# facebookresearch/omni3d

Hardware: AMD Instinct MI355X
Metric: images/sec train DLA34_FPN b=4/GPU (higher is better)
Workload: dtype f32; 1 GPU; cubercnn_DLA34_FPN train step, batch 4/GPU, synthetic Omni3D 512x512 (8 GT/img), fwd+10 losses+bwd+allreduce+divergence guard+SGD, random-init weights; global_batch=4, image=512x512, parallelism=dp1 (flat-bucket RCCL all-reduce)

## Files before the change

### include/omni3d_hip.h

```cpp
#ifndef OMNI3D_HIP_H
#define OMNI3D_HIP_H

#ifdef __cplusplus
extern "C" {
#endif


int omni_iou_box3d(const float* boxes1, int N, const float* boxes2, int M, const int* valid1, float* vol,
                   float* iou, int* overflow, void* stream);

int omni_iou_box3d_pairs(const float* boxes1, const float* boxes2, const int* idx1, const int* idx2,
                         long long npairs, const int* valid1, float* vol, float* iou, int* overflow,
                         void* stream);

int omni_iou_box3d_pairs_algo(const float* boxes1, const float* boxes2, const int* idx1, const int* idx2,
                              long long npairs, const int* valid1, float* vol, float* iou, int* overflow,
                              int lanes_per_pair, void* stream);

int omni_box3d_validity(const float* boxes, int N, float eps_coplanar, float eps_nonzero, int* valid,
                        int* counts, void* stream);

int omni_nms3d(const float* verts, const float* score, const int* cls, const int* count, int B, int S, float iou_thr,
               int class_agnostic, float eps_coplanar, float eps_nonzero, float* iou, int* keep, int* order, int* new_count,
               int* overflow, void* stream);
// ... 142 lines not shown


int omni_pairwise_iou(const float* boxes1, int N, const float* boxes2, int M, int mode, float* out, void* stream);


int omni_rpn_finalize_labels(const float* anchors, int A, int B, const int* gt_off, const float* ign,
                             const int* ign_off, const signed char* match_label, const int* gt_best_idx,
                             const float* pos_val, const int* pos_idx, const float* neg_val, const int* neg_idx,
                             int kpos, int kneg, int batch_per_image, float ignore_thresh, signed char* labels,
                             int* counts, void* stream);

int omni_rpn_gather_logits(const void* const* level_ptrs, const int* level_hw, int nlev, int B, float* logits,
                           void* stream);

int omni_rpn_head16_fwd(const void* const* t, const long long* pix, int nlev, const float* w_obj, const float* b_obj,
                        const float* w_del, const float* b_del, const void* const* y, void* stream);
int omni_rpn_head16_dgrad(const void* const* dy, const void* const* t, const long long* pix, int nlev, const float* w_obj,
                          const float* w_del, int relu_mask, const void* const* dt, void* stream);
int omni_rpn_head16_wgrad(const void* const* dy, const void* const* t, const long long* pix, int nlev, float* partial,
                          int partial_rows, float* dw_obj, float* db_obj, float* dw_del, float* db_del, int accumulate, void* stream);

int omni_rpn_loss_fwd(const void* const* level_ptrs, const int* level_hw, int nlev, int B, const float* anchors,
                      const signed char* labels, const int* matched_idx, const float* gt, const int* gt_off,
                      double* sums, void* stream);
int omni_rpn_loss_bwd(const void* const* level_ptrs, const void* const* dlevel_ptrs, const int* level_hw, int nlev,
                      int B, const float* anchors, const signed char* labels, const int* matched_idx,
                      const float* gt, const int* gt_off, const float* g_cls, const float* g_loc, float inv_norm,
                      void* stream);

int omni_rpn_loss_plain_fwd(const void* const* level_ptrs, const int* level_hw, int nlev, int B, const float* anchors,
                            const signed char* labels, const int* matched_idx, const float* gt, const int* gt_off,
                            double* sums, void* stream);
int omni_rpn_loss_plain_bwd(const void* const* level_ptrs, const void* const* dlevel_ptrs, const int* level_hw, int nlev,
                            int B, const float* anchors, const signed char* labels, const int* matched_idx,
                            const float* gt, const int* gt_off, const float* g_cls, const float* g_loc, float inv_norm,
                            void* stream);

int omni_rpn_reg_loss_fwd(const void* const* level_ptrs, const int* level_hw, int nlev, int B, const float* anchors,
                          const signed char* labels, const int* matched_idx, const float* gt, const int* gt_off, int plain,
                          int reg_type, float beta, float scale_clamp, double* sums, void* stream);
int omni_rpn_reg_loss_bwd(const void* const* level_ptrs, const void* const* dlevel_ptrs, const int* level_hw, int nlev,
                          int B, const float* anchors, const signed char* labels, const int* matched_idx,
                          const float* gt, const int* gt_off, int plain, int reg_type, float beta, float scale_clamp,
                          const float* g_cls, const float* g_loc, float inv_norm, void* stream);

int omni_rpn_decode(const void* const* level_ptrs, const int* level_hw, int nlev, int B, int Ktot,
                    const int* slot_level, const int* idx, const float* anchors, const int* image_hw,
                    float scale_clamp, float min_size, float* boxes, int* valid, void* stream);

int omni_rpn_mask_scores(const float* scores, const int* keep, long long n, float* masked, void* stream);
int omni_rpn_collect(const float* boxes, const float* top_v, const int* top_i, int B, int N, int P, float* prop,
                     int* count, void* stream);

int omni_rpn_match_draw(const float* anchors, int A, const float* gt, const int* gt_off, int B, int G, float thr_lo,
                        float thr_hi, int l0, int l1, int l2, int allow_low_quality, const float* expo, long long* draw_state,
                        int* ticket, float eps, float* matched_val, int* matched_idx, signed char* match_label, int* gt_best_bits,
                        int* gt_best_idx, float* key_pos, float* key_neg, void* stream);
int omni_roi_sample_draw(const float* prop_boxes, const int* prop_count, int B, int pmax, const float* gt, const int* gt_cls,
                         const int* gt_off, const float* ign, const int* ign_off, const float* expo, long long* draw_state, int* ticket,
                         float iou_thr, float ignore_thresh, float eps, int num_classes, int batch_per_image, int nfg_max,
                         int append_gt, float* out_boxes, int* out_cls, int* out_gt, float* out_iou, int* out_counts, int* out_row,
                         int first, float* first_boxes, int* first_cls, int* first_row, void* stream);


int omni_roi_levels(const float* rois, int R, int min_level, int max_level, float canonical_size,
                    int canonical_level, int* levels, void* stream);

int omni_roi_align_fwd(const void* const* level_ptrs, const int* level_hw, const float* level_scale, int nlev,
                       const float* rois, const int* batch_idx, const int* levels, int R, int P, int C,
                       float* out, void* stream);
int omni_roi_align_fwd_mode(const void* const* level_ptrs, const int* level_hw, const float* level_scale, int nlev,
                            const float* rois, const int* batch_idx, const int* levels, int R, int P, int C, int aligned, float* out,
                            void* stream);
int omni_roi_align_bwd_mode(const void* const* dlevel_ptrs, const int* level_hw, const float* level_scale, int nlev,
                            const float* rois, const int* batch_idx, const int* levels, int R, int P, int C, int aligned,
                            const float* dout, void* stream);
int omni_roi_pool_fwd(const void* const* level_ptrs, const int* level_hw, const float* level_scale, int nlev, const float* rois,
                      const int* batch_idx, const int* levels, int R, int P, int C, float* out, int* argmax, void* stream);
int omni_roi_pool_bwd(const void* const* dlevel_ptrs, const int* level_hw, const float* level_scale, int nlev, const int* batch_idx,
                      const int* levels, int R, int P, int C, const float* dout, const int* argmax, void* stream);
int omni_roi_align_fwd2(const void* const* level_ptrs, const int* level_hw, const float* level_scale, int nlev,
                        const float* rois, const int* batch_idx, const int* levels, int R, int P, int C, float* out,
                        float* out2, int per_image, int first, void* stream);
int omni_roi_align_bwd(const void* const* dlevel_ptrs, const int* level_hw, const float* level_scale, int nlev,
                       const float* rois, const int* batch_idx, const int* levels, int R, int P, int C,
                       const float* dout, void* stream);
int omni_roi_align_bwd2(const void* const* dlevel_ptrs, const int* level_hw, const float* level_scale, int nlev,
                        const float* rois, const int* batch_idx, const int* levels, int R, int P, int C,
                        const float* dout, const float* dout2, int per_image, int first, void* stream);
int omni_roi_align_bwd_det(const void* const* dlevel_ptrs, const int* level_hw, const float* level_scale, int nlev, int B,
                           const float* rois, const int* batch_idx, const int* levels, int R, int P, int C, const float* dout,
                           const float* dout2, int per_image, int first, float* ws, long long ws_floats, int* ctr, int n_ctr,
                           long long* plan, void* stream);


int omni_box_loss_fwd(const float* pred, int ldp, int R, int K, const int* cls, const float* prop, const float* gt,
                      const int* gt_row, float wx, float wy, float ww, float wh, double* sums, void* stream);
int omni_box_loss_bwd(const float* pred, int ldp, int R, int K, const int* cls, const float* prop, const float* gt,
                      const int* gt_row, float wx, float wy, float ww, float wh, const double* sums,
                      const float* g_cls, const float* g_reg, float* dpred, void* stream);

int omni_box_reg_loss_fwd(const float* pred, int ldp, int R, int K, const int* cls, const float* prop, const float* gt,
                          const int* gt_row, float wx, float wy, float ww, float wh, int reg_type, float beta,
                          float scale_clamp, double* sums, void* stream);
int omni_box_reg_loss_bwd(const float* pred, int ldp, int R, int K, const int* cls, const float* prop, const float* gt,
                          const int* gt_row, float wx, float wy, float ww, float wh, int reg_type, float beta,
                          float scale_clamp, const double* sums, const float* g_cls, const float* g_reg, float* dpred,
                          void* stream);

int omni_box_decode_gt_class(const float* pred, int ldp, int R, int K, const int* cls, const float* prop, float wx, float wy,
                             float ww, float wh, float scale_clamp, float* out, void* stream);

int omni_cube_loss_fwd(const float* head, int ldh, int F, int K, int mode, int bins, const float* zscales, const float* zstats,
                       const float* boxes, const int* cls, const int* img,
                       const float* Ks, const float* v2r, const float* priors, const float* gt3d,
                       const float* gtpose, const int* gt_row, float w_dims, float w_pose, float w_xy, float w_z, float w_joint,
                       float* vals, float* jac, float* red, void* stream);
int omni_cube_loss_bwd(const float* vals, const float* jac, const float* red, const float* gk, const int* cls,
                       const float* boxes, int F, int K, int mode, int bins, const float* zscales, int ldh, float* dhead,
                       void* stream);
int omni_cube_decode(const float* head, int ldh, int F, int K, int mode, int bins, const float* zscales, const float* zstats,
                     const float* boxes, const int* cls, const int* img,
                     const float* Ks, const float* v2r, const float* ratio, const float* priors, float* cube3d,
                     float* pose, float* verts, void* stream);
int omni_cuboid_corners(const float* box3d, const float* R, int n, float* verts, void* stream);

int omni_conv2d_fwd_stats(const float* x, const float* w, float* out, int N, int H, int W, int C, int K, int R, int S,
                          int stride, int pad, int ldx, int ldo, float* stats, int stats_rows, int* nblk_out, void* stream);
int omni_wino_out_stats(const float* M, float* y, int N, int H, int W, int K, int tile, float* stats, int stats_rows,
                        int* nblk_out, void* stream);
int omni_wino_out_bn_bwd_stats(const float* M, float* y, int N, int H, int W, int K, int tile, const float* bn_x,
                               const float* mean_rstd, const float* scale_shift, float* stats, int stats_rows, int* nblk_out,
                               void* stream);
int omni_stem_conv_fwd_stats(const float* x, const float* w, float* out, int N, int H, int W, int C, int K, int R, int ldx,
                             int ldo, float* stats, int stats_rows, int* nblk_out, void* stream);

int omni_gemm_engine(const float* A, const float* B, float* C, const float* bias, int form, int batch, int M, int N, int K,
                     int lda, int ldb, int ldc, long long stride_a, long long stride_b, long long stride_c, int splits,
                     int relu, int accumulate, int tile, int workgroups, void* stream);
int omni_gemm_engine_det(const float* A, const float* B, float* C, const float* bias, int form, int batch, int M, int N, int K,
                         int lda, int ldb, int ldc, long long stride_a, long long stride_b, long long stride_c, int splits,
                         int relu, int accumulate, int tile, int workgroups, float* ws, long long ws_floats, int* ctr, int n_ctr,
                         long long* plan, void* stream);

int omni_transpose2d(const float* src, float* dst, int rows, int cols, void* stream);

int omni_det_scores(const float* pred, int ld, const float* rois, const int* count, const int* image_hw, int B, int P, int K,
                    float wx, float wy, float ww, float wh, float score_thresh, float* scores, float* probs, float* boxes,
                    void* stream);
int omni_det_nms_boxes(const float* boxes, const float* vals, const int* idx, int B, int PK, int K, int cap, float* nms_boxes,
                       int* valid, void* stream);
int omni_det_compact(const int* keep, const int* valid, const float* vals, const int* idx, const float* boxes, int B, int PK,
                     int K, int cap, int topk, float* out_box, float* out_score, int* out_cls, int* out_roi, int* out_count,
                     void* stream);

int omni_resize_bilinear_u8(const unsigned char* src, unsigned char* dst, unsigned char* tmp, int planes, int H, int W,
                            int HO, int WO, const int* bounds_h, const int* kk_h, int ksize_h, const int* bounds_v,
                            const int* kk_v, int ksize_v, int flip, void* stream);


int omni_sgd_step(float* param, const float* grad, float* momentum_buf, long long n, float lr, float momentum,
                  float dampening, float weight_decay, int nesterov, int first_step, float grad_scale,
                  const float* skip_flag, void* stream);
int omni_adam_step(float* param, const float* grad, float* exp_avg, float* exp_avg_sq, float* max_exp_avg_sq, long long n, float lr,
                   float beta1, float beta2, float eps, float weight_decay, int decoupled, const float* step, float grad_scale,
                   const float* skip_flag, void* stream);
// ... 149 lines not shown
```

### omni3d_amd/csrc/roi_align.hip

```cpp
#include <device_rt.h>
#pragma clang fp contract(off)

namespace {

constexpr int MAXL = 8;
struct FeatLevels {
    float* f[MAXL];
    int H[MAXL], W[MAXL];
    float scale[MAXL];
    int nlev;
};

__global__ void roi_levels_kernel(const float* __restrict__ rois, int R, int min_level, int max_level,
                                  float canonical_size, int canonical_level, int* __restrict__ levels) {
    const int r = blockIdx.x * blockDim.x + threadIdx.x;
    if (r >= R) return;
    const float w = rois[4 * r + 2] - rois[4 * r + 0], h = rois[4 * r + 3] - rois[4 * r + 1];
    const float sz = sqrtf(w * h);
    float lv = floorf((float)canonical_level + log2f(sz / canonical_size + 1e-8f));
    lv = fminf(fmaxf(lv, (float)min_level), (float)max_level);
    levels[r] = (int)lv - min_level;
}

struct Tap { int y0, y1, x0, x1; float w00, w01, w10, w11; bool ok; };

__device__ __forceinline__ Tap make_tap(float y, float x, int H, int W) {
    Tap t;
    t.ok = !(y < -1.0f || y > (float)H || x < -1.0f || x > (float)W);
    if (y <= 0.f) y = 0.f;
    if (x <= 0.f) x = 0.f;
    int y_low = (int)y, x_low = (int)x, y_high, x_high;
    if (y_low >= H - 1) { y_high = y_low = H - 1; y = (float)y_low; } else { y_high = y_low + 1; }
    if (x_low >= W - 1) { x_high = x_low = W - 1; x = (float)x_low; } else { x_high = x_low + 1; }
    const float ly = y - (float)y_low, lx = x - (float)x_low, hy = 1.f - ly, hx = 1.f - lx;
    t.y0 = y_low; t.y1 = y_high; t.x0 = x_low; t.x1 = x_high;
    t.w00 = hy * hx; t.w01 = hy * lx; t.w10 = ly * hx; t.w11 = ly * lx;
    return t;
}

template <int DIR>
__global__ void __launch_bounds__(256) roi_align_kernel(FeatLevels fl, const float* __restrict__ rois,
                                                        const int* __restrict__ batch_idx, const int* __restrict__ levels,
                                                        int R, int P, int C, float* __restrict__ out,
                                                        float* __restrict__ out2 = nullptr, int per_image = 0, int first = 0, int aligned = 1) {
    const int wave = threadIdx.x >> 6, lane = threadIdx.x & 63;
    const long job = (long)blockIdx.x * 4 + wave;
    if (job >= (long)R * P * P) return;
    const int r = (int)(job / (P * P)), bin = (int)(job % (P * P));
    const int ph = bin / P, pw = bin % P;
    const int l = levels[r];
    const int H = fl.H[l], W = fl.W[l];
    const float sc = fl.scale[l];
    const float off = aligned ? 0.5f : 0.f;
    const float sw = rois[4 * r + 0] * sc - off, sh = rois[4 * r + 1] * sc - off;
    const float ew = rois[4 * r + 2] * sc - off, eh = rois[4 * r + 3] * sc - off;
    float rw = ew - sw, rh = eh - sh;
    if (!aligned) { rw = fmaxf(rw, 1.f); rh = fmaxf(rh, 1.f); }
    const float bin_h = rh / (float)P, bin_w = rw / (float)P;
    const int gh = (int)ceilf(rh / (float)P), gw = (int)ceilf(rw / (float)P);
    const float count = (float)max(gh * gw, 1);
    float* feat = fl.f[l] + (long)batch_idx[r] * H * W * C;
    float* o = out + job * C;
    if (DIR == 1) {
        for (int c = lane; c < C; c += 64) {
            const float g = o[c] / count;
            for (int iy = 0; iy < gh; ++iy) {
                const float y = sh + (float)ph * bin_h + ((float)iy + 0.5f) * bin_h / (float)gh;
                for (int ix = 0; ix < gw; ++ix) {
                    const float x = sw + (float)pw * bin_w + ((float)ix + 0.5f) * bin_w / (float)gw;
                    const Tap t = make_tap(y, x, H, W);
                    if (!t.ok) continue;
                    atomicAdd(feat + ((long)t.y0 * W + t.x0) * C + c, g * t.w00);
                    atomicAdd(feat + ((long)t.y0 * W + t.x1) * C + c, g * t.w01);
                    atomicAdd(feat + ((long)t.y1 * W + t.x0) * C + c, g * t.w10);
                    atomicAdd(feat + ((long)t.y1 * W + t.x1) * C + c, g * t.w11);
                }
            }
        }
        return;
    }
    const int C4 = C >> 2;
    for (int c4 = lane; c4 < C4; c4 += 64) {
        float4 acc = make_float4(0.f, 0.f, 0.f, 0.f);
        for (int iy = 0; iy < gh; ++iy) {
            const float y = sh + (float)ph * bin_h + ((float)iy + 0.5f) * bin_h / (float)gh;
            for (int ix = 0; ix < gw; ++ix) {
                const float x = sw + (float)pw * bin_w + ((float)ix + 0.5f) * bin_w / (float)gw;
                const Tap t = make_tap(y, x, H, W);
                if (!t.ok) continue;
                const float* p00 = feat + ((long)t.y0 * W + t.x0) * C + 4 * c4;
                const float* p01 = feat + ((long)t.y0 * W + t.x1) * C + 4 * c4;
                const float* p10 = feat + ((long)t.y1 * W + t.x0) * C + 4 * c4;
                const float* p11 = feat + ((long)t.y1 * W + t.x1) * C + 4 * c4;
                const float4 a = *reinterpret_cast<const float4*>(p00), b = *reinterpret_cast<const float4*>(p01);
                const float4 c = *reinterpret_cast<const float4*>(p10), d = *reinterpret_cast<const float4*>(p11);
                acc.x += t.w00 * a.x + t.w01 * b.x + t.w10 * c.x + t.w11 * d.x;
                acc.y += t.w00 * a.y + t.w01 * b.y + t.w10 * c.y + t.w11 * d.y;
                acc.z += t.w00 * a.z + t.w01 * b.z + t.w10 * c.z + t.w11 * d.z;
                acc.w += t.w00 * a.w + t.w01 * b.w + t.w10 * c.w + t.w11 * d.w;
            }
        }
        acc.x /= count; acc.y /= count; acc.z /= count; acc.w /= count;
        *reinterpret_cast<float4*>(o + 4 * c4) = acc;
        if (DIR == 0 && out2 != nullptr && (r % per_image) < first)
            *reinterpret_cast<float4*>(out2 + (((long)(r / per_image) * first + (r % per_image)) * P * P + bin) * C + 4 * c4) = acc;
    }
}

constexpr int SEP_MAXF = 144;

struct Tap1 { int lo, hi; float wlo, whi; bool ok; };
__device__ __forceinline__ Tap1 make_tap1(float v, int L) {
    Tap1 t;
    t.ok = !(v < -1.0f || v > (float)L);
    if (v <= 0.f) v = 0.f;
    int lo = (int)v, hi;
    if (lo >= L - 1) { hi = lo = L - 1; v = (float)lo; } else { hi = lo + 1; }
    const float l = v - (float)lo;
    t.lo = lo; t.hi = hi; t.whi = l; t.wlo = 1.f - l;
    return t;
}

template <int PP>
__global__ void __launch_bounds__(256) roi_align_bwd_sep_kernel(FeatLevels fl, const float* __restrict__ rois,
                                                                const int* __restrict__ batch_idx,
                                                                const int* __restrict__ levels, int R, int C,
                                                                const float* __restrict__ dout, const float* __restrict__ dout2,
                                                                int per_image, int first) {
    __shared__ __attribute__((aligned(16))) float s_w[4][2][SEP_MAXF][8];
    const int wave = threadIdx.x >> 6, lane = threadIdx.x & 63;
    const int CG = (C + 63) / 64;
    const long job = (long)blockIdx.x * 4 + wave;
    const bool live = job < (long)R * CG;
    const int r = live ? (int)(job / CG) : 0, cg = live ? (int)(job % CG) : 0;
    const int c = cg * 64 + lane;
    const int l = levels[r];
    const int H = fl.H[l], W = fl.W[l];
    const float sc = fl.scale[l];
    const float sw = rois[4 * r + 0] * sc - 0.5f, sh = rois[4 * r + 1] * sc - 0.5f;
    const float ew = rois[4 * r + 2] * sc - 0.5f, eh = rois[4 * r + 3] * sc - 0.5f;
    const float rw = ew - sw, rh = eh - sh;
    const float bin_h = rh / (float)PP, bin_w = rw / (float)PP;
    const int gh = (int)ceilf(rh / (float)PP), gw = (int)ceilf(rw / (float)PP);
    const bool any = live && gh > 0 && gw > 0;
    float* feat = fl.f[l] + (long)batch_idx[r] * H * W * C;
    int Y0 = 0, X0 = 0, fh = 0, fw = 0;
    if (any) {
        Y0 = make_tap1(sh + 0.5f * bin_h / (float)gh, H).lo;
        X0 = make_tap1(sw + 0.5f * bin_w / (float)gw, W).lo;
        fh = make_tap1(sh + (float)(PP - 1) * bin_h + ((float)(gh - 1) + 0.5f) * bin_h / (float)gh, H).hi - Y0 + 1;
        fw = make_tap1(sw + (float)(PP - 1) * bin_w + ((float)(gw - 1) + 0.5f) * bin_w / (float)gw, W).hi - X0 + 1;
    }
    const bool sep = any && fh <= SEP_MAXF && fw <= SEP_MAXF;
    float (*wy)[8] = s_w[wave][0];
    float (*wx)[8] = s_w[wave][1];
    if (sep) {
        for (int i = lane; i < fh * 8; i += 64) wy[i >> 3][i & 7] = 0.f;
        for (int i = lane; i < fw * 8; i += 64) wx[i >> 3][i & 7] = 0.f;
    }
    __syncthreads();
    if (sep) {
        if (lane < PP) {
            for (int ix = 0; ix < gw; ++ix) {
                const Tap1 t = make_tap1(sw + (float)lane * bin_w + ((float)ix + 0.5f) * bin_w / (float)gw, W);
                if (!t.ok) continue;
                wx[t.lo - X0][lane] += t.wlo;
                wx[t.hi - X0][lane] += t.whi;
            }
        } else if (lane >= 32 && lane < 32 + PP) {
            const int ph = lane - 32;
            for (int iy = 0; iy < gh; ++iy) {
                const Tap1 t = make_tap1(sh + (float)ph * bin_h + ((float)iy + 0.5f) * bin_h / (float)gh, H);
                if (!t.ok) continue;
                wy[t.lo - Y0][ph] += t.wlo;
                wy[t.hi - Y0][ph] += t.whi;
            }
        }
    }
    __syncthreads();
    if (!any || c >= C) return;
    const float inv_count = 1.f / (float)(gh * gw);
    const float* o = dout != nullptr ? dout + (long)r * PP * PP * C + c : nullptr;
    const float* o2 = nullptr;
    if (dout2 != nullptr) {
        const int img = r / per_image, k = r - img * per_image;
        if (k < first) o2 = dout2 + ((long)img * first + k) * PP * PP * C + c;
    }
    auto gval = [&](int bin) -> float {
        float v = o != nullptr ? o[(long)bin * C] : 0.f;
        if (o2 != nullptr) v += o2[(long)bin * C];
        return v * inv_count;
    };
    if (sep) {
        float g[PP][PP];
#pragma unroll
        for (int ph = 0; ph < PP; ++ph)
#pragma unroll
            for (int pw = 0; pw < PP; ++pw) g[ph][pw] = gval(ph * PP + pw);
        for (int yy = 0; yy < fh; ++yy) {
            float rowT[PP];
#pragma unroll
            for (int pw = 0; pw < PP; ++pw) rowT[pw] = 0.f;
            bool row_any = false;
// ... 212 lines not shown
    if (wave == 0 && cok) {
        float* feat = fl.f[l] + (long)n * H * W * C + c;
#pragma unroll
        for (int yy = 0; yy < GT_TH; ++yy)
#pragma unroll
            for (int xx = 0; xx < GT_TW; ++xx)
                if (ty0 + yy < H && tx0 + xx < W) *reinterpret_cast<float4*>(feat + ((long)(ty0 + yy) * W + tx0 + xx) * C) = acc[yy * GT_TW + xx];
    }
}

FeatLevels make_feat(const void* const* ptrs, const int* hw, const float* scales, int nlev) {
    FeatLevels fl;
    for (int l = 0; l < MAXL; ++l) { fl.f[l] = nullptr; fl.H[l] = fl.W[l] = 0; fl.scale[l] = 0.f; }
    for (int l = 0; l < nlev; ++l) { fl.f[l] = (float*)ptrs[l]; fl.H[l] = hw[2 * l]; fl.W[l] = hw[2 * l + 1]; fl.scale[l] = scales[l]; }
    fl.nlev = nlev;
    return fl;
}

template <int DIR>
__global__ void __launch_bounds__(256) roi_pool_kernel(FeatLevels fl, const float* __restrict__ rois, const int* __restrict__ batch_idx,
                                                       const int* __restrict__ levels, int R, int P, int C, float* __restrict__ out,
                                                       int* __restrict__ argmax) {
    const int wave = threadIdx.x >> 6, lane = threadIdx.x & 63;
    const long job = (long)blockIdx.x * 4 + wave;
    if (job >= (long)R * P * P) return;
    const int r = (int)(job / (P * P)), bin = (int)(job % (P * P));
    const int ph = bin / P, pw = bin % P;
    const int l = levels[r];
    const int H = fl.H[l], W = fl.W[l];
    float* feat = fl.f[l] + (long)batch_idx[r] * H * W * C;
    const int C4 = C >> 2;
    if (DIR == 1) {
        for (int c4 = lane; c4 < C4; c4 += 64) {
            const float4 g = *reinterpret_cast<const float4*>(out + job * C + 4 * c4);
            const int4 a = *reinterpret_cast<const int4*>(argmax + job * C + 4 * c4);
            if (a.x >= 0) atomicAdd(feat + (long)a.x * C + 4 * c4 + 0, g.x);
            if (a.y >= 0) atomicAdd(feat + (long)a.y * C + 4 * c4 + 1, g.y);
            if (a.z >= 0) atomicAdd(feat + (long)a.z * C + 4 * c4 + 2, g.z);
            if (a.w >= 0) atomicAdd(feat + (long)a.w * C + 4 * c4 + 3, g.w);
        }
        return;
    }
    const float sc = fl.scale[l];
    const int rsw = (int)roundf(rois[4 * r + 0] * sc), rsh = (int)roundf(rois[4 * r + 1] * sc);
    const int rew = (int)roundf(rois[4 * r + 2] * sc), reh = (int)roundf(rois[4 * r + 3] * sc);
    const int rw = max(rew - rsw + 1, 1), rh = max(reh - rsh + 1, 1);
    const float bh = (float)rh / (float)P, bw = (float)rw / (float)P;
    int hs = (int)floorf((float)ph * bh), he = (int)ceilf((float)(ph + 1) * bh);
    int ws = (int)floorf((float)pw * bw), we = (int)ceilf((float)(pw + 1) * bw);
    hs = min(max(hs + rsh, 0), H); he = min(max(he + rsh, 0), H);
    ws = min(max(ws + rsw, 0), W); we = min(max(we + rsw, 0), W);
    const bool empty = he <= hs || we <= ws;
    for (int c4 = lane; c4 < C4; c4 += 64) {
        const float init = empty ? 0.f : -3.402823466e+38f;
        float4 m = make_float4(init, init, init, init);
        int4 a = make_int4(-1, -1, -1, -1);
        for (int h = hs; h < he; ++h)
            for (int w = ws; w < we; ++w) {
                const int idx = h * W + w;
                const float4 v = *reinterpret_cast<const float4*>(feat + (long)idx * C + 4 * c4);
                if (v.x > m.x) { m.x = v.x; a.x = idx; }
                if (v.y > m.y) { m.y = v.y; a.y = idx; }
                if (v.z > m.z) { m.z = v.z; a.z = idx; }
                if (v.w > m.w) { m.w = v.w; a.w = idx; }
            }
        *reinterpret_cast<float4*>(out + job * C + 4 * c4) = m;
        *reinterpret_cast<int4*>(argmax + job * C + 4 * c4) = a;
    }
}

}

extern "C" {

int omni_roi_levels(const float* rois, int R, int min_level, int max_level, float canonical_size, int canonical_level,
                    int* levels, void* stream) {
    if (R < 0 || max_level < min_level) return OMNI_ERR_ARG;
    if (R == 0) return OMNI_OK;
    hipLaunchKernelGGL(roi_levels_kernel, dim3((R + 255) / 256), dim3(256), 0, (hipStream_t)stream, rois, R, min_level,
                       max_level, canonical_size, canonical_level, levels);
    return omni_launch_status();
}

int omni_roi_align_fwd(const void* const* level_ptrs, const int* level_hw, const float* level_scale, int nlev,
                       const float* rois, const int* batch_idx, const int* levels, int R, int P, int C, float* out,
                       void* stream) {
    if (nlev <= 0 || nlev > MAXL || (C & 3) || P <= 0) return OMNI_ERR_ARG;
    if (R == 0) return OMNI_OK;
    FeatLevels fl = make_feat(level_ptrs, level_hw, level_scale, nlev);
    const long jobs = (long)R * P * P;
    hipLaunchKernelGGL(HIP_KERNEL_NAME(roi_align_kernel<0>), dim3((unsigned)((jobs + 3) / 4)), dim3(256), 0,
                       (hipStream_t)stream, fl, rois, batch_idx, levels, R, P, C, out);
    return omni_launch_status();
}

int omni_roi_align_fwd2(const void* const* level_ptrs, const int* level_hw, const float* level_scale, int nlev,
                        const float* rois, const int* batch_idx, const int* levels, int R, int P, int C, float* out,
                        float* out2, int per_image, int first, void* stream) {
    if (nlev <= 0 || nlev > MAXL || (C & 3) || P <= 0) return OMNI_ERR_ARG;
    if (out2 != nullptr && (per_image <= 0 || first < 0 || first > per_image || R % per_image != 0)) return OMNI_ERR_ARG;
    if (R == 0) return OMNI_OK;
    FeatLevels fl = make_feat(level_ptrs, level_hw, level_scale, nlev);
    const long jobs = (long)R * P * P;
    hipLaunchKernelGGL(HIP_KERNEL_NAME(roi_align_kernel<0>), dim3((unsigned)((jobs + 3) / 4)), dim3(256), 0,
                       (hipStream_t)stream, fl, rois, batch_idx, levels, R, P, C, out, out2, per_image, first);
    return omni_launch_status();
}

int omni_roi_align_fwd_mode(const void* const* level_ptrs, const int* level_hw, const float* level_scale, int nlev,
                            const float* rois, const int* batch_idx, const int* levels, int R, int P, int C, int aligned, float* out,
                            void* stream) {
    if (nlev <= 0 || nlev > MAXL || (C & 3) || P <= 0) return OMNI_ERR_ARG;
    if (R == 0) return OMNI_OK;
    FeatLevels fl = make_feat(level_ptrs, level_hw, level_scale, nlev);
    const long jobs = (long)R * P * P;
    hipLaunchKernelGGL(HIP_KERNEL_NAME(roi_align_kernel<0>), dim3((unsigned)((jobs + 3) / 4)), dim3(256), 0,
                       (hipStream_t)stream, fl, rois, batch_idx, levels, R, P, C, out, (float*)nullptr, 0, 0, aligned != 0);
    return omni_launch_status();
}
int omni_roi_align_bwd_mode(const void* const* dlevel_ptrs, const int* level_hw, const float* level_scale, int nlev,
                            const float* rois, const int* batch_idx, const int* levels, int R, int P, int C, int aligned,
                            const float* dout, void* stream) {
    if (nlev <= 0 || nlev > MAXL || (C & 3) || P <= 0 || dout == nullptr) return OMNI_ERR_ARG;
    if (R == 0) return OMNI_OK;
    FeatLevels fl = make_feat(dlevel_ptrs, level_hw, level_scale, nlev);
    const long jobs = (long)R * P * P;
    hipLaunchKernelGGL(HIP_KERNEL_NAME(roi_align_kernel<1>), dim3((unsigned)((jobs + 3) / 4)), dim3(256), 0,
                       (hipStream_t)stream, fl, rois, batch_idx, levels, R, P, C, const_cast<float*>(dout), (float*)nullptr, 0, 0, aligned != 0);
    return omni_launch_status();
}

int omni_roi_pool_fwd(const void* const* level_ptrs, const int* level_hw, const float* level_scale, int nlev, const float* rois,
                      const int* batch_idx, const int* levels, int R, int P, int C, float* out, int* argmax, void* stream) {
    if (nlev <= 0 || nlev > MAXL || (C & 3) || P <= 0 || out == nullptr || argmax == nullptr) return OMNI_ERR_ARG;
    if (R == 0) return OMNI_OK;
    FeatLevels fl = make_feat(level_ptrs, level_hw, level_scale, nlev);
    const long jobs = (long)R * P * P;
    hipLaunchKernelGGL(HIP_KERNEL_NAME(roi_pool_kernel<0>), dim3((unsigned)((jobs + 3) / 4)), dim3(256), 0, (hipStream_t)stream, fl, rois,
                       batch_idx, levels, R, P, C, out, argmax);
    return omni_launch_status();
}
int omni_roi_pool_bwd(const void* const* dlevel_ptrs, const int* level_hw, const float* level_scale, int nlev, const int* batch_idx,
                      const int* levels, int R, int P, int C, const float* dout, const int* argmax, void* stream) {
    if (nlev <= 0 || nlev > MAXL || (C & 3) || P <= 0 || dout == nullptr || argmax == nullptr) return OMNI_ERR_ARG;
    if (R == 0) return OMNI_OK;
    FeatLevels fl = make_feat(dlevel_ptrs, level_hw, level_scale, nlev);
    const long jobs = (long)R * P * P;
    hipLaunchKernelGGL(HIP_KERNEL_NAME(roi_pool_kernel<1>), dim3((unsigned)((jobs + 3) / 4)), dim3(256), 0, (hipStream_t)stream, fl,
                       (const float*)nullptr, batch_idx, levels, R, P, C, const_cast<float*>(dout), const_cast<int*>(argmax));
    return omni_launch_status();
}

static int roi_align_bwd_impl(const void* const* dlevel_ptrs, const int* level_hw, const float* level_scale, int nlev,
                              const float* rois, const int* batch_idx, const int* levels, int R, int P, int C, const float* dout,
                              const float* dout2, int per_image, int first, void* stream) {
    if (nlev <= 0 || nlev > MAXL || (C & 3) || P <= 0 || (dout == nullptr && dout2 == nullptr)) return OMNI_ERR_ARG;
    if (dout2 != nullptr && (per_image <= 0 || first < 0 || first > per_image || R % per_image != 0)) return OMNI_ERR_ARG;
    if (R == 0) return OMNI_OK;
    FeatLevels fl = make_feat(dlevel_ptrs, level_hw, level_scale, nlev);
    if (P == 7) {
        const long jobs = (long)R * ((C + 63) / 64);
        hipLaunchKernelGGL(HIP_KERNEL_NAME(roi_align_bwd_sep_kernel<7>), dim3((unsigned)((jobs + 3) / 4)), dim3(256), 0,
                           (hipStream_t)stream, fl, rois, batch_idx, levels, R, C, dout, dout2, per_image, first);
        return omni_launch_status();
    }
    if (dout == nullptr || dout2 != nullptr) return OMNI_ERR_ARG;
    const long jobs = (long)R * P * P;
    hipLaunchKernelGGL(HIP_KERNEL_NAME(roi_align_kernel<1>), dim3((unsigned)((jobs + 3) / 4)), dim3(256), 0,
                       (hipStream_t)stream, fl, rois, batch_idx, levels, R, P, C, const_cast<float*>(dout));
    return omni_launch_status();
}

int omni_roi_align_bwd_det(const void* const* dlevel_ptrs, const int* level_hw, const float* level_scale, int nlev, int B,
                           const float* rois, const int* batch_idx, const int* levels, int R, int P, int C, const float* dout,
                           const float* dout2, int per_image, int first, float* ws, long long ws_floats, int* ctr, int n_ctr,
                           long long* plan, void* stream) {
    (void)ctr; (void)n_ctr;
    if (nlev <= 0 || nlev > MAXL || (C & 3) || C > 256 || P != 7 || B <= 0 || B > 255 || R < 0 || R > GT_MAXR || (dout == nullptr && dout2 == nullptr)) return OMNI_ERR_ARG;
    if (dout2 != nullptr && (per_image <= 0 || first < 0 || first > per_image || R % per_image != 0)) return OMNI_ERR_ARG;
    FeatLevels fl = make_feat(dlevel_ptrs, level_hw, level_scale, nlev);
    GatherTiles gt;
    int total = 0;
    for (int l = 0; l < MAXL; ++l) {
        gt.off[l] = total;
        gt.tx[l] = gt.ty[l] = gt.px[l] = gt.py[l] = 1;
        if (l < nlev) {
            if (fl.H[l] > 65535 || fl.W[l] > 65535) return OMNI_ERR_ARG;
            gt.tx[l] = (fl.W[l] + GT_TW - 1) / GT_TW;
            gt.ty[l] = (fl.H[l] + GT_TH - 1) / GT_TH;
            gt.px[l] = (gt.tx[l] + GT_PW - 1) / GT_PW;
            gt.py[l] = (gt.ty[l] + GT_PH - 1) / GT_PH;
            const long patches = (long)B * gt.px[l] * gt.py[l];
            if (total + patches > (1L << 22)) return OMNI_ERR_ARG;
            total += (int)patches;
        }
    }
    for (int l = nlev; l <= MAXL; ++l) gt.off[l] = total;
    gt.B = B;
    const long long need = 8LL * R + 4;
    if (plan != nullptr) { plan[0] = plan[1] = plan[2] = 0; plan[3] = need; return OMNI_OK; }
    if (total == 0) return OMNI_OK;
// ... 26 lines not shown
```

### omni3d_amd/kernels/det.py

```python
import collections
import ctypes
import math

import torch

from .. import lib as _lib
from . import detmode as _det
from . import select as _select

_P = ctypes.c_void_p


def _ptrs(tensors):
    arr = (ctypes.c_void_p * len(tensors))(*[t.data_ptr() for t in tensors])
    return arr


def _ints(vals):
    return (ctypes.c_int * len(vals))(*[int(v) for v in vals])


def _floats(vals):
    return (ctypes.c_float * len(vals))(*[float(v) for v in vals])

# ... 207 lines not shown
    first = int(min(first, batch_per_image))
    f_boxes = _empty((B, first, 4), torch.float32, prop_boxes) if first > 0 else None
    f_cls = _empty((B, first), torch.int32, prop_boxes) if first > 0 else None
    f_row = _empty((B, first), torch.int32, prop_boxes) if first > 0 else None
    state, ticket = draw.tensors(prop_boxes.device) if expo is None else (None, None)
    L.call("omni_roi_sample_draw", _lib.ptr(prop_boxes), _lib.ptr(prop_count), B, pmax, _lib.ptr(gt), _lib.ptr(gt_cls),
           _lib.ptr(gt_off), _lib.ptr(ign), _lib.ptr(ign_off), _lib.ptr(expo), _lib.ptr(state), _lib.ptr(ticket), float(iou_thr),
           float(ignore_thresh), float(eps), int(num_classes), int(batch_per_image), int(batch_per_image * positive_fraction),
           int(append_gt), _lib.ptr(o_boxes), _lib.ptr(o_cls), _lib.ptr(o_gt), _lib.ptr(o_iou), _lib.ptr(o_cnt), _lib.ptr(o_row), first,
           _lib.ptr(f_boxes), _lib.ptr(f_cls), _lib.ptr(f_row), _lib.stream_of(prop_boxes))
    return o_boxes, o_cls, o_gt, o_iou, o_cnt, o_row, (f_boxes, f_cls, f_row)


def roi_levels(rois, min_level=2, max_level=6, canonical_size=224.0, canonical_level=4):
    L = _dev(rois)
    R = rois.shape[0]
    lv = _empty((R,), torch.int32, rois)
    L.call("omni_roi_levels", _lib.ptr(rois), R, min_level, max_level, float(canonical_size), canonical_level, _lib.ptr(lv),
           _lib.stream_of(rois))
    return lv


def _feat_args(feats_nhwc, scales):
    p = _ptrs(feats_nhwc)
    hw = _ints([v for t in feats_nhwc for v in (t.shape[1], t.shape[2])])
    sc = _floats(scales)
    return (p, hw, sc), (_cast(p), _cast(hw), _cast(sc), len(feats_nhwc))


def roi_align_fwd(feats_nhwc, scales, rois, batch_idx, levels, P):
    L = _dev(rois, batch_idx, levels, *feats_nhwc)
    R, C = rois.shape[0], feats_nhwc[0].shape[3]
    out = _empty((R, P, P, C), torch.float32, rois)
    keep, a = _feat_args(feats_nhwc, scales)
    L.call("omni_roi_align_fwd", *a, _lib.ptr(rois), _lib.ptr(batch_idx), _lib.ptr(levels), R, P, C, _lib.ptr(out),
           _lib.stream_of(rois))
    return out


def roi_align_fwd_mode(feats_nhwc, scales, rois, batch_idx, levels, P, aligned):
    L = _dev(rois, batch_idx, levels, *feats_nhwc)
    R, C = rois.shape[0], feats_nhwc[0].shape[3]
    out = _empty((R, P, P, C), torch.float32, rois)
    keep, a = _feat_args(feats_nhwc, scales)
    L.call("omni_roi_align_fwd_mode", *a, _lib.ptr(rois), _lib.ptr(batch_idx), _lib.ptr(levels), R, P, C, int(bool(aligned)), _lib.ptr(out),
           _lib.stream_of(rois))
    return out


def roi_align_bwd_mode(dfeats_nhwc, scales, rois, batch_idx, levels, P, aligned, dout):
    L = _dev(rois, batch_idx, levels, dout, *dfeats_nhwc)
    R, C = rois.shape[0], dfeats_nhwc[0].shape[3]
    keep, a = _feat_args(dfeats_nhwc, scales)
    L.call("omni_roi_align_bwd_mode", *a, _lib.ptr(rois), _lib.ptr(batch_idx), _lib.ptr(levels), R, P, C, int(bool(aligned)), _lib.ptr(dout),
           _lib.stream_of(rois))


def roi_pool_fwd(feats_nhwc, scales, rois, batch_idx, levels, P):
    L = _dev(rois, batch_idx, levels, *feats_nhwc)
    R, C = rois.shape[0], feats_nhwc[0].shape[3]
    out = _empty((R, P, P, C), torch.float32, rois)
    arg = _empty((R, P, P, C), torch.int32, rois)
    keep, a = _feat_args(feats_nhwc, scales)
    L.call("omni_roi_pool_fwd", *a, _lib.ptr(rois), _lib.ptr(batch_idx), _lib.ptr(levels), R, P, C, _lib.ptr(out), _lib.ptr(arg),
           _lib.stream_of(rois))
    return out, arg


def roi_pool_bwd(dfeats_nhwc, scales, batch_idx, levels, P, dout, argmax):
    L = _dev(batch_idx, levels, dout, argmax, *dfeats_nhwc)
    R, C = dout.shape[0], dfeats_nhwc[0].shape[3]
    keep, a = _feat_args(dfeats_nhwc, scales)
    L.call("omni_roi_pool_bwd", *a, _lib.ptr(batch_idx), _lib.ptr(levels), R, P, C, _lib.ptr(dout), _lib.ptr(argmax), _lib.stream_of(dout))


def roi_align_fwd2(feats_nhwc, scales, rois, batch_idx, levels, P, per_image, first):
    L = _dev(rois, batch_idx, levels, *feats_nhwc)
    R, C = rois.shape[0], feats_nhwc[0].shape[3]
    out = _empty((R, P, P, C), torch.float32, rois)
    out2 = _empty(((R // per_image) * first, P, P, C), torch.float32, rois)
    keep, a = _feat_args(feats_nhwc, scales)
    L.call("omni_roi_align_fwd2", *a, _lib.ptr(rois), _lib.ptr(batch_idx), _lib.ptr(levels), R, P, C, _lib.ptr(out), _lib.ptr(out2),
           int(per_image), int(first), _lib.stream_of(rois))
    return out, out2


def roi_align_bwd_deterministic(P, R, C=256):
    return _det.on() and P == 7 and R <= 4096 and C <= 256


def roi_align_bwd_det(dfeats_nhwc, scales, rois, batch_idx, levels, P, dout, dout2=None, per_image=0, first=0):
    L = _dev(rois, batch_idx, levels, dout, dout2, *dfeats_nhwc)
    R, C, B = rois.shape[0], dfeats_nhwc[0].shape[3], dfeats_nhwc[0].shape[0]
    keep, a = _feat_args(dfeats_nhwc, scales)
    assert (dout is None or dout.is_contiguous()) and (dout2 is None or dout2.is_contiguous())
    _det.plan_launch(L, "omni_roi_align_bwd_det", rois, (*a, B, _lib.ptr(rois), _lib.ptr(batch_idx), _lib.ptr(levels), R, P, C, _lib.ptr(dout),
                                                         _lib.ptr(dout2), int(per_image), int(first)))


def roi_align_bwd(dfeats_nhwc, scales, rois, batch_idx, levels, P, dout, dout2=None, per_image=0, first=0):
    L = _dev(rois, batch_idx, levels, dout, dout2, *dfeats_nhwc)
    R, C = rois.shape[0], dfeats_nhwc[0].shape[3]
    keep, a = _feat_args(dfeats_nhwc, scales)
    if dout2 is None:
        L.call("omni_roi_align_bwd", *a, _lib.ptr(rois), _lib.ptr(batch_idx), _lib.ptr(levels), R, P, C, _lib.ptr(dout),
               _lib.stream_of(rois))
        return
    assert dout2.is_contiguous() and (dout is None or dout.is_contiguous())
    L.call("omni_roi_align_bwd2", *a, _lib.ptr(rois), _lib.ptr(batch_idx), _lib.ptr(levels), R, P, C, _lib.ptr(dout), _lib.ptr(dout2),
           int(per_image), int(first), _lib.stream_of(rois))


def box_loss_fwd(pred, K, cls, prop, gt, gt_row, weights=(10.0, 10.0, 5.0, 5.0), reg_type="smooth_l1", beta=0.0, scale_clamp=SCALE_CLAMP):
    L = _dev(pred, cls, prop, gt, gt_row)
    R, ldp = pred.shape
    sums = _empty((7,), torch.float64, pred)
    reg = box_reg_args(reg_type, beta, scale_clamp)
    L.call("omni_box_loss_fwd" if reg is None else "omni_box_reg_loss_fwd", _lib.ptr(pred), ldp, R, K, _lib.ptr(cls), _lib.ptr(prop), _lib.ptr(gt),
           _lib.ptr(gt_row), *[float(w) for w in weights], *(reg or ()), _lib.ptr(sums), _lib.stream_of(pred))
    return sums


def box_loss_bwd(pred, K, cls, prop, gt, gt_row, sums, g_cls, g_reg, weights=(10.0, 10.0, 5.0, 5.0), reg_type="smooth_l1", beta=0.0,
                 scale_clamp=SCALE_CLAMP):
    L = _dev(pred, cls, prop, gt, gt_row, sums, g_cls, g_reg)
    R, ldp = pred.shape
    dpred = torch.empty_like(pred)
    reg = box_reg_args(reg_type, beta, scale_clamp)
    L.call("omni_box_loss_bwd" if reg is None else "omni_box_reg_loss_bwd", _lib.ptr(pred), ldp, R, K, _lib.ptr(cls), _lib.ptr(prop), _lib.ptr(gt),
           _lib.ptr(gt_row), *[float(w) for w in weights], *(reg or ()), _lib.ptr(sums), _lib.ptr(g_cls), _lib.ptr(g_reg), _lib.ptr(dpred),
           _lib.stream_of(pred))
    return dpred


def box_decode_gt_class(pred, K, cls, prop, weights=(10.0, 10.0, 5.0, 5.0), scale_clamp=4.135166556742356):
    L = _dev(pred, cls, prop)
    R, ldp = pred.shape
    out = _empty((R, 4), torch.float32, pred)
    L.call("omni_box_decode_gt_class", _lib.ptr(pred), ldp, R, K, _lib.ptr(cls), _lib.ptr(prop), *[float(w) for w in weights],
           float(scale_clamp), _lib.ptr(out), _lib.stream_of(pred))
    return out


def train_vis_pick(pred, head, uncert_off, rois, cls, nfg, K, weights=(10.0, 10.0, 5.0, 5.0), scale_clamp=4.135166556742356, iou_thr=0.5,
                   max_keep=20):
    L = _dev(pred, head, rois, cls, nfg)
    B, Fc = cls.shape
    if B == 0 or pred.shape[0] % B or head.shape[0] != B * Fc or tuple(rois.shape) != (B, Fc, 4) or tuple(nfg.shape) != (B,):
        raise ValueError(f"train_vis_pick: pred {tuple(pred.shape)}, head {tuple(head.shape)}, rois {tuple(rois.shape)}, nfg "
                         f"{tuple(nfg.shape)} do not describe {B} images of {Fc} cube rows")
    S, ldp, ldh = pred.shape[0] // B, pred.shape[1], head.shape[1]
    keep_row = _empty((B, max_keep), torch.int32, pred)
    keep_count = _empty((B,), torch.int32, pred)
    keep_box = _empty((B, max_keep, 4), torch.float32, pred)
    keep_score = _empty((B, max_keep), torch.float32, pred)
    L.call("omni_train_vis_pick", _lib.ptr(pred), ldp, _lib.ptr(head), ldh, int(uncert_off), _lib.ptr(rois), _lib.ptr(cls), _lib.ptr(nfg),
           B, S, Fc, int(K), *[float(w) for w in weights], float(scale_clamp), float(iou_thr), int(max_keep), _lib.ptr(keep_row),
           _lib.ptr(keep_count), _lib.ptr(keep_box), _lib.ptr(keep_score), _lib.stream_of(pred))
    return keep_row, keep_count, keep_box, keep_score


NMS3D_METHODS = ("evaluator", "exact")
NMS3D_MAX_SLOTS = 1024


def nms3d(verts, scores, cls, count, iou_thr, class_agnostic=True, eps_coplanar=1e-4, eps_nonzero=1e-8, method="evaluator"):
# ... 258 lines not shown
```

### omni3d_amd/lib.py

```python
import ctypes
import os

import torch

_HERE = os.path.dirname(os.path.abspath(__file__))
LIB_PATH = os.path.join(_HERE, "libomni3d_hip" + os.environ.get("OMNI_LIB_SUFFIX", "") + ".so")

_P, _I, _L, _F, _D = ctypes.c_void_p, ctypes.c_int, ctypes.c_longlong, ctypes.c_float, ctypes.c_double
_CODES = {"p": _P, "i": _I, "l": _L, "f": _F, "d": _D}

HEADER_PATH = os.path.join(os.path.dirname(_HERE), "include", "omni3d_hip.h")


def parse_header(path=HEADER_PATH):
    import re
    text = open(path).read()
    text = re.sub(r"/\*.*?\*/", "", text, flags=re.S)
    decls = {}
    for m in re.finditer(r"\bint\s+(omni_\w+)\s*\(([^)]*)\)\s*;", text):
        codes = ""
        for arg in m.group(2).split(","):
            a = " ".join(arg.replace("const", " ").split())
            if "*" in a:
                codes += "p"
            elif a.startswith("long long"):
                codes += "l"
            elif a.startswith("float"):
                codes += "f"
            elif a.startswith("double"):
                codes += "d"
            elif a.startswith("int"):
                codes += "i"
            else:
                raise ValueError(f"unparsed argument {arg!r} in {m.group(1)}")
        decls[m.group(1)] = codes
    return decls


SIGNATURES = parse_header()


class OmniHipError(RuntimeError):
    pass


class HipLibrary:
    def __init__(self, path, emulated=False):
        if not os.path.exists(path):
            raise OmniHipError(
                f"{path} not found: build it with `make -C omni3d_amd/csrc` (hipcc, gfx950). "
                "omni3d_amd has no CPU fallback."
            )
        self.path = path
        self.emulated = emulated
        self._dll = ctypes.CDLL(path)
        self._fn = {}
        for name, codes in SIGNATURES.items():
            fn = getattr(self._dll, name)
            fn.argtypes = [_CODES[c] for c in codes]
            fn.restype = ctypes.c_int
            self._fn[name] = fn

    def call(self, name, *args):
        rc = self._fn[name](*args)
        if rc != 0:
            raise OmniHipError(f"{name} failed with status {rc}")


_lib = None


def get():
    global _lib
    if _lib is None:
        _lib = HipLibrary(LIB_PATH)
    return _lib


def _install_for_tests(lib):
    global _lib
    _lib = lib


def ptr(t):
    return None if t is None else t.data_ptr()


def stream_of(t):
    if t.is_cuda:
        return torch.cuda.current_stream(t.device).cuda_stream
    return None


def check_device(*tensors):
    lib = get()
    for t in tensors:
        if t is None:
            continue
        if not t.is_cuda and not lib.emulated:
            raise OmniHipError("omni3d_amd ops run on the GPU only (got a CPU tensor); there is no CPU path")
        if not t.is_contiguous():
            raise OmniHipError("omni3d_amd ops need contiguous tensors")
    return lib
```

Measured before the change: 383.7 images/s.

## Add per-ROI block ROI-align forward kernel with shared-memory axis tap tables

```diff
diff --git a/include/omni3d_hip.h b/include/omni3d_hip.h
--- a/include/omni3d_hip.h
+++ b/include/omni3d_hip.h
@@ -248,6 +248,10 @@
 int omni_roi_align_fwd2(const void* const* level_ptrs, const int* level_hw, const float* level_scale, int nlev,
                         const float* rois, const int* batch_idx, const int* levels, int R, int P, int C, float* out,
                         float* out2, int per_image, int first, void* stream);
+int omni_roi_align_fwd_algo(const void* const* level_ptrs, const int* level_hw, const float* level_scale, int nlev,
+                            const float* rois, const int* batch_idx, const int* levels, int R, int P, int C, int aligned, float* out,
+                            float* out2, int per_image, int first, int algo, void* stream);
+int omni_roi_align_fwd_table_cap(void);
 int omni_roi_align_bwd(const void* const* dlevel_ptrs, const int* level_hw, const float* level_scale, int nlev,
                        const float* rois, const int* batch_idx, const int* levels, int R, int P, int C,
                        const float* dout, void* stream);
diff --git a/omni3d_amd/csrc/roi_align.hip b/omni3d_amd/csrc/roi_align.hip
--- a/omni3d_amd/csrc/roi_align.hip
+++ b/omni3d_amd/csrc/roi_align.hip
@@ -39,14 +39,10 @@
 }
 
 template <int DIR>
-__global__ void __launch_bounds__(256) roi_align_kernel(FeatLevels fl, const float* __restrict__ rois,
-                                                        const int* __restrict__ batch_idx, const int* __restrict__ levels,
-                                                        int R, int P, int C, float* __restrict__ out,
-                                                        float* __restrict__ out2 = nullptr, int per_image = 0, int first = 0, int aligned = 1) {
-    const int wave = threadIdx.x >> 6, lane = threadIdx.x & 63;
-    const long job = (long)blockIdx.x * 4 + wave;
-    if (job >= (long)R * P * P) return;
-    const int r = (int)(job / (P * P)), bin = (int)(job % (P * P));
+__device__ __forceinline__ void roi_align_bin(const FeatLevels& fl, const float* __restrict__ rois, const int* __restrict__ batch_idx,
+                                              const int* __restrict__ levels, int r, int bin, int lane, int P, int C,
+                                              float* __restrict__ out, float* __restrict__ out2, int per_image, int first, int aligned) {
+    const long job = (long)r * (P * P) + bin;
     const int ph = bin / P, pw = bin % P;
     const int l = levels[r];
     const int H = fl.H[l], W = fl.W[l];
@@ -107,6 +103,17 @@
     }
 }
 
+template <int DIR>
+__global__ void __launch_bounds__(256) roi_align_kernel(FeatLevels fl, const float* __restrict__ rois,
+                                                        const int* __restrict__ batch_idx, const int* __restrict__ levels,
+                                                        int R, int P, int C, float* __restrict__ out,
+                                                        float* __restrict__ out2 = nullptr, int per_image = 0, int first = 0, int aligned = 1) {
+    const int wave = threadIdx.x >> 6, lane = threadIdx.x & 63;
+    const long job = (long)blockIdx.x * 4 + wave;
+    if (job >= (long)R * P * P) return;
+    roi_align_bin<DIR>(fl, rois, batch_idx, levels, (int)(job / (P * P)), (int)(job % (P * P)), lane, P, C, out, out2, per_image, first, aligned);
+}
+
 constexpr int SEP_MAXF = 144;
 
 struct Tap1 { int lo, hi; float wlo, whi; bool ok; };
@@ -119,6 +126,123 @@
     const float l = v - (float)lo;
     t.lo = lo; t.hi = hi; t.whi = l; t.wlo = 1.f - l;
     return t;
+}
+
+constexpr int FWD_TAB_CAP = 126;
+
+struct alignas(16) AxisTap { int lo, hi; float wlo, whi; };
+
+__device__ __forceinline__ void fill_axis_taps(AxisTap* __restrict__ tab, int t, int nt, int P, int g, float start, float bin, int L, int stride) {
+    for (int e = t; e < P * g; e += nt) {
+        const int p = e / g, i = e - p * g;
+        const Tap1 tp = make_tap1(start + (float)p * bin + ((float)i + 0.5f) * bin / (float)g, L);
+        AxisTap a;
+        a.lo = tp.ok ? tp.lo * stride : -1;
+        a.hi = tp.ok ? tp.hi * stride : -1;
+        a.wlo = tp.wlo; a.whi = tp.whi;
+        tab[e] = a;
+    }
+}
+
+__device__ __forceinline__ void add_sample(float4& acc, const AxisTap& y, const AxisTap& x, const float4& a, const float4& b,
+                                           const float4& c, const float4& d) {
+    const float w00 = y.wlo * x.wlo, w01 = y.wlo * x.whi, w10 = y.whi * x.wlo, w11 = y.whi * x.whi;
+    acc.x += w00 * a.x + w01 * b.x + w10 * c.x + w11 * d.x;
+    acc.y += w00 * a.y + w01 * b.y + w10 * c.y + w11 * d.y;
+    acc.z += w00 * a.z + w01 * b.z + w10 * c.z + w11 * d.z;
+    acc.w += w00 * a.w + w01 * b.w + w10 * c.w + w11 * d.w;
+}
+
+__device__ __forceinline__ float4 load_tap(const char* __restrict__ img, unsigned byte_off) {
+    return *reinterpret_cast<const float4*>(img + byte_off);
+}
+
+#ifndef OMNI_ROI_FWD_WAVES
+#define OMNI_ROI_FWD_WAVES 4
+#endif
+#ifndef OMNI_ROI_FWD_SPLIT
+#define OMNI_ROI_FWD_SPLIT 1
+#endif
+constexpr int FWD_NW = OMNI_ROI_FWD_WAVES;
+constexpr int FWD_SPLIT = OMNI_ROI_FWD_SPLIT;
+constexpr int FWD_V = FWD_NW * FWD_SPLIT;
+
+__global__ void __launch_bounds__(64 * FWD_NW) OMNI_WAVES_PER_EU(8) roi_align_fwd_table_kernel(FeatLevels fl, const float* __restrict__ rois,
+                                                                  const int* __restrict__ batch_idx, const int* __restrict__ levels,
+                                                                  int R, int P, int C, float* __restrict__ out, float* __restrict__ out2,
+                                                                  int per_image, int first, int aligned) {
+    __shared__ AxisTap s_tap[2][FWD_TAB_CAP];
+    const int tid = threadIdx.x, lane = tid & 63;
+    const int wave = __float_as_int(omni_readlane(__int_as_float(tid >> 6), 0));
+    const int r = blockIdx.x / FWD_SPLIT, v0 = (blockIdx.x % FWD_SPLIT) * FWD_NW + wave;
+    const int l = levels[r];
+    const int H = fl.H[l], W = fl.W[l];
+    const float sc = fl.scale[l];
+    const float off = aligned ? 0.5f : 0.f;
+    const float sw = rois[4 * r + 0] * sc - off, sh = rois[4 * r + 1] * sc - off;
+    const float ew = rois[4 * r + 2] * sc - off, eh = rois[4 * r + 3] * sc - off;
+    float rw = ew - sw, rh = eh - sh;
+    if (!aligned) { rw = fmaxf(rw, 1.f); rh = fmaxf(rh, 1.f); }
+    const float bin_h = rh / (float)P, bin_w = rw / (float)P;
+    const int gh = (int)ceilf(rh / (float)P), gw = (int)ceilf(rw / (float)P);
+    const float count = (float)max(gh * gw, 1);
+    const bool empty = gh <= 0 || gw <= 0;
+    const int gmax = FWD_TAB_CAP / P;
+    const int PP = P * P;
+    if (!empty && (gh > gmax || gw > gmax)) {
+        for (int bin = v0; bin < PP; bin += FWD_V) roi_align_bin<0>(fl, rois, batch_idx, levels, r, bin, lane, P, C, out, out2, per_image, first, aligned);
+        return;
+    }
+    if (!empty) {
+        if (wave < FWD_NW / 2) fill_axis_taps(s_tap[0], tid, 32 * FWD_NW, P, gh, sh, bin_h, H, W * C * 4);
+        else fill_axis_taps(s_tap[1], tid - 32 * FWD_NW, 32 * FWD_NW, P, gw, sw, bin_w, W, C * 4);
+    }
+    __syncthreads();
+    const int nh = empty ? 0 : gh, nw = empty ? 0 : gw, n = nh * nw;
+    const char* img = reinterpret_cast<const char*>(fl.f[l] + (long)batch_idx[r] * H * W * C);
+    float* o = out + (long)r * PP * C;
+    float* o2 = nullptr;
+    if (out2 != nullptr && (r % per_image) < first) o2 = out2 + ((long)(r / per_image) * first + (r % per_image)) * PP * C;
+    const int C4 = C >> 2;
+    int ph = v0 / P, pw = v0 % P;
+    for (int bin = v0; bin < PP; bin += FWD_V) {
+        const AxisTap* ty = s_tap[0] + ph * nh;
+        const AxisTap* tx = s_tap[1] + pw * nw;
+        for (int c4 = lane; c4 < C4; c4 += 64) {
+            const unsigned cb = 16u * (unsigned)c4;
+            float4 acc = make_float4(0.f, 0.f, 0.f, 0.f);
+            int iy = 0, ix = 0;
+            for (int s = 0; s < n; s += 2) {
+                const AxisTap y0 = ty[iy], x0 = tx[ix];
+                if (++ix == nw) { ix = 0; ++iy; }
+                const bool two = s + 1 < n;
+                const AxisTap y1 = ty[two ? iy : 0], x1 = tx[two ? ix : 0];
+                if (++ix == nw) { ix = 0; ++iy; }
+                const bool ok0 = (y0.lo | x0.lo) >= 0, ok1 = two && (y1.lo | x1.lo) >= 0;
+                if (ok0 && ok1) {
+                    const float4 a0 = load_tap(img, (unsigned)(y0.lo + x0.lo) + cb), b0 = load_tap(img, (unsigned)(y0.lo + x0.hi) + cb);
+                    const float4 c0 = load_tap(img, (unsigned)(y0.hi + x0.lo) + cb), d0 = load_tap(img, (unsigned)(y0.hi + x0.hi) + cb);
+                    const float4 a1 = load_tap(img, (unsigned)(y1.lo + x1.lo) + cb), b1 = load_tap(img, (unsigned)(y1.lo + x1.hi) + cb);
+                    const float4 c1 = load_tap(img, (unsigned)(y1.hi + x1.lo) + cb), d1 = load_tap(img, (unsigned)(y1.hi + x1.hi) + cb);
+                    add_sample(acc, y0, x0, a0, b0, c0, d0);
+                    add_sample(acc, y1, x1, a1, b1, c1, d1);
+                } else if (ok0) {
+                    const float4 a0 = load_tap(img, (unsigned)(y0.lo + x0.lo) + cb), b0 = load_tap(img, (unsigned)(y0.lo + x0.hi) + cb);
+                    const float4 c0 = load_tap(img, (unsigned)(y0.hi + x0.lo) + cb), d0 = load_tap(img, (unsigned)(y0.hi + x0.hi) + cb);
+                    add_sample(acc, y0, x0, a0, b0, c0, d0);
+                } else if (ok1) {
+                    const float4 a1 = load_tap(img, (unsigned)(y1.lo + x1.lo) + cb), b1 = load_tap(img, (unsigned)(y1.lo + x1.hi) + cb);
+                    const float4 c1 = load_tap(img, (unsigned)(y1.hi + x1.lo) + cb), d1 = load_tap(img, (unsigned)(y1.hi + x1.hi) + cb);
+                    add_sample(acc, y1, x1, a1, b1, c1, d1);
+                }
+            }
+            acc.x /= count; acc.y /= count; acc.z /= count; acc.w /= count;
+            *reinterpret_cast<float4*>(o + (long)bin * C + 4 * c4) = acc;
+            if (o2 != nullptr) *reinterpret_cast<float4*>(o2 + (long)bin * C + 4 * c4) = acc;
+        }
+        pw += FWD_V;
+        while (pw >= P) { pw -= P; ++ph; }
+    }
 }
 
 template <int PP>
@@ -497,41 +621,42 @@
     return omni_launch_status();
 }
 
+int omni_roi_align_fwd_algo(const void* const* level_ptrs, const int* level_hw, const float* level_scale, int nlev,
+                            const float* rois, const int* batch_idx, const int* levels, int R, int P, int C, int aligned, float* out,
+                            float* out2, int per_image, int first, int algo, void* stream) {
+    if (nlev <= 0 || nlev > MAXL || (C & 3) || P <= 0 || R < 0 || (algo != 0 && algo != 1)) return OMNI_ERR_ARG;
+    if (out2 != nullptr && (per_image <= 0 || first < 0 || first > per_image || R % per_image != 0)) return OMNI_ERR_ARG;
+    if (R == 0) return OMNI_OK;
+    FeatLevels fl = make_feat(level_ptrs, level_hw, level_scale, nlev);
+    for (int l = 0; l < nlev; ++l)
+        if ((long)fl.H[l] * fl.W[l] * C * 4 > 0x7fffffffL) algo = 0;
+    if (algo == 1) {
+        hipLaunchKernelGGL(roi_align_fwd_table_kernel, dim3((unsigned)R * FWD_SPLIT), dim3(64 * FWD_NW), 0, (hipStream_t)stream, fl, rois, batch_idx, levels,
+                           R, P, C, out, out2, per_image, first, aligned != 0);
+        return omni_launch_status();
+    }
+    const long jobs = (long)R * P * P;
+    hipLaunchKernelGGL(HIP_KERNEL_NAME(roi_align_kernel<0>), dim3((unsigned)((jobs + 3) / 4)), dim3(256), 0,
+                       (hipStream_t)stream, fl, rois, batch_idx, levels, R, P, C, out, out2, per_image, first, aligned != 0);
+    return omni_launch_status();
+}
+int omni_roi_align_fwd_table_cap(void) { return FWD_TAB_CAP; }
+
 int omni_roi_align_fwd(const void* const* level_ptrs, const int* level_hw, const float* level_scale, int nlev,
                        const float* rois, const int* batch_idx, const int* levels, int R, int P, int C, float* out,
                        void* stream) {
-    if (nlev <= 0 || nlev > MAXL || (C & 3) || P <= 0) return OMNI_ERR_ARG;
-    if (R == 0) return OMNI_OK;
-    FeatLevels fl = make_feat(level_ptrs, level_hw, level_scale, nlev);
-    const long jobs = (long)R * P * P;
-    hipLaunchKernelGGL(HIP_KERNEL_NAME(roi_align_kernel<0>), dim3((unsigned)((jobs + 3) / 4)), dim3(256), 0,
-                       (hipStream_t)stream, fl, rois, batch_idx, levels, R, P, C, out);
-    return omni_launch_status();
-}
-
+    return omni_roi_align_fwd_algo(level_ptrs, level_hw, level_scale, nlev, rois, batch_idx, levels, R, P, C, 1, out, nullptr, 0, 0, 1, stream);
+}
 int omni_roi_align_fwd2(const void* const* level_ptrs, const int* level_hw, const float* level_scale, int nlev,
                         const float* rois, const int* batch_idx, const int* levels, int R, int P, int C, float* out,
                         float* out2, int per_image, int first, void* stream) {
-    if (nlev <= 0 || nlev > MAXL || (C & 3) || P <= 0) return OMNI_ERR_ARG;
-    if (out2 != nullptr && (per_image <= 0 || first < 0 || first > per_image || R % per_image != 0)) return OMNI_ERR_ARG;
-    if (R == 0) return OMNI_OK;
-    FeatLevels fl = make_feat(level_ptrs, level_hw, level_scale, nlev);
-    const long jobs = (long)R * P * P;
-    hipLaunchKernelGGL(HIP_KERNEL_NAME(roi_align_kernel<0>), dim3((unsigned)((jobs + 3) / 4)), dim3(256), 0,
-                       (hipStream_t)stream, fl, rois, batch_idx, levels, R, P, C, out, out2, per_image, first);
-    return omni_launch_status();
+    return omni_roi_align_fwd_algo(level_ptrs, level_hw, level_scale, nlev, rois, batch_idx, levels, R, P, C, 1, out, out2, per_image, first, 1, stream);
 }
 
 int omni_roi_align_fwd_mode(const void* const* level_ptrs, const int* level_hw, const float* level_scale, int nlev,
                             const float* rois, const int* batch_idx, const int* levels, int R, int P, int C, int aligned, float* out,
                             void* stream) {
-    if (nlev <= 0 || nlev > MAXL || (C & 3) || P <= 0) return OMNI_ERR_ARG;
-    if (R == 0) return OMNI_OK;
-    FeatLevels fl = make_feat(level_ptrs, level_hw, level_scale, nlev);
-    const long jobs = (long)R * P * P;
-    hipLaunchKernelGGL(HIP_KERNEL_NAME(roi_align_kernel<0>), dim3((unsigned)((jobs + 3) / 4)), dim3(256), 0,
-                       (hipStream_t)stream, fl, rois, batch_idx, levels, R, P, C, out, (float*)nullptr, 0, 0, aligned != 0);
-    return omni_launch_status();
+    return omni_roi_align_fwd_algo(level_ptrs, level_hw, level_scale, nlev, rois, batch_idx, levels, R, P, C, aligned, out, nullptr, 0, 0, 1, stream);
 }
 int omni_roi_align_bwd_mode(const void* const* dlevel_ptrs, const int* level_hw, const float* level_scale, int nlev,
                             const float* rois, const int* batch_idx, const int* levels, int R, int P, int C, int aligned,
diff --git a/omni3d_amd/kernels/det.py b/omni3d_amd/kernels/det.py
--- a/omni3d_amd/kernels/det.py
+++ b/omni3d_amd/kernels/det.py
@@ -313,6 +313,22 @@
     keep, a = _feat_args(feats_nhwc, scales)
     L.call("omni_roi_align_fwd2", *a, _lib.ptr(rois), _lib.ptr(batch_idx), _lib.ptr(levels), R, P, C, _lib.ptr(out), _lib.ptr(out2),
            int(per_image), int(first), _lib.stream_of(rois))
+    return out, out2
+
+
+def roi_align_fwd_table_cap():
+    return int(_lib.get()._fn["omni_roi_align_fwd_table_cap"]())
+
+
+def roi_align_fwd_algo(feats_nhwc, scales, rois, batch_idx, levels, P, algo, aligned=True, out=None, out2=None, per_image=0, first=0):
+    L = _dev(rois, batch_idx, levels, out, out2, *feats_nhwc)
+    R, C = rois.shape[0], feats_nhwc[0].shape[3]
+    if out is None:
+        out = _empty((R, P, P, C), torch.float32, rois)
+    assert tuple(out.shape) == (R, P, P, C) and (out2 is None or tuple(out2.shape) == ((R // per_image) * first, P, P, C))
+    keep, a = _feat_args(feats_nhwc, scales)
+    L.call("omni_roi_align_fwd_algo", *a, _lib.ptr(rois), _lib.ptr(batch_idx), _lib.ptr(levels), R, P, C, int(bool(aligned)), _lib.ptr(out),
+           _lib.ptr(out2), int(per_image), int(first), int(algo), _lib.stream_of(rois))
     return out, out2
 
 
diff --git a/omni3d_amd/lib.py b/omni3d_amd/lib.py
--- a/omni3d_amd/lib.py
+++ b/omni3d_amd/lib.py
@@ -21,6 +21,8 @@
         codes = ""
         for arg in m.group(2).split(","):
             a = " ".join(arg.replace("const", " ").split())
+            if a == "void" and "," not in m.group(2):
+                continue
             if "*" in a:
                 codes += "p"
             elif a.startswith("long long"):
```

New measurement: 381.5 images/s. No clear change (-0.6%).
